# llm-d/llm-d-workload-variant-autoscaler

Measured on AMD Instinct MI355X. Metric: desired-replica accuracy + SLO-attainment %, Llama-3-8B synthetic QPS ramp, higher is better.
Workload: dtype bf16; 1 GPU; model=meta-llama/Llama-3.1-8B, global_batch=256, seq_len=150, parallelism=dp1, device=AMD Radeon Graphics

## Files before the change

### wva_amd/calibration/model.py

```python
from __future__ import annotations

import math
from dataclasses import dataclass
from typing import List, Optional

import torch

from .. import ops


@dataclass
class LlamaConfig:
    name: str = "llama"
    hidden_size: int = 4096
    intermediate_size: int = 14336
    num_layers: int = 32
    num_q_heads: int = 32
    num_kv_heads: int = 8
    head_dim: int = 128
    vocab_size: int = 128256
    rope_theta: float = 500000.0
    rms_eps: float = 1e-5

    @property
# ... 144 lines not shown
        self.context_lens[:batch] = context_len
        for layer in range(self.cfg.num_layers):
            if self.cache_dtype == torch.bfloat16:
                self.k_cache[layer][:batch, :, :context_len].normal_(0.0, 1.0)
                self.v_cache[layer][:batch, :, :context_len].normal_(0.0, 1.0)
            else:
                shape = self.k_cache[layer][:batch, :, :context_len].shape
                for cache in (self.k_cache, self.v_cache):
                    cache[layer][:batch, :, :context_len] = torch.randn(
                        shape, device=self.device, dtype=torch.bfloat16
                    ).to(self.cache_dtype)

    def _linear(self, x: torch.Tensor, layer, name: str) -> torch.Tensor:
        if self.weights_dtype == "bf16":
            w = getattr(layer, name) if layer is not None else self.lm_head
            return ops.linear(x, w)
        w8, w_scale = (
            getattr(layer, name + "_q") if layer is not None else self.lm_head_q
        )
        if not x.is_cuda:
            return (
                x.float() @ (w8.float() * w_scale[:, None]).t()
            ).to(x.dtype)
        if x.shape[0] <= 64 and x.shape[1] % 128 == 0:
            from .. import ops as _ops

            return _ops._require_ext().skinny_linear_fp8(x, w8, w_scale)
        return (x @ (w8.to(x.dtype) * w_scale[:, None].to(x.dtype)).t())

    @torch.no_grad()
    def decode_step(self, token_ids: torch.Tensor) -> torch.Tensor:
        cfg = self.cfg
        B = token_ids.shape[0]
        positions = self.context_lens[:B].clone()

        ctx = positions + 1
        x = self.embed.index_select(0, token_ids)
        residual: Optional[torch.Tensor] = None

        for li, layer in enumerate(self.layers):
            if residual is None:
                residual = x.clone()
                h = ops.rmsnorm(x, layer.input_norm, None, cfg.rms_eps)
            else:
                h = ops.rmsnorm(x, layer.input_norm, residual, cfg.rms_eps)

            qkv = self._linear(h, layer, "wqkv")
            q = ops.rope_append_kv(
                qkv, self.k_cache[li][:B], self.v_cache[li][:B],
                positions, cfg.num_q_heads, cfg.num_kv_heads, cfg.rope_theta,
            )

            attn = ops.gqa_decode_attn(
                q, self.k_cache[li][:B], self.v_cache[li][:B], ctx, self.scale
            )
            x = self._linear(attn.reshape(B, cfg.q_size), layer, "wo")

            h2 = ops.rmsnorm(x, layer.post_attn_norm, residual, cfg.rms_eps)
            gate_up = self._linear(h2, layer, "w_gate_up")
            act = ops.silu_mul_fused(gate_up)
            x = self._linear(act, layer, "w_down")

        final = ops.rmsnorm(x, self.final_norm, residual, cfg.rms_eps)
        logits = self._linear(final, None, "lm_head")
        self.context_lens[:B] += 1
        return logits

    @torch.no_grad()
    def prefill(self, token_ids: torch.Tensor) -> torch.Tensor:
        cfg = self.cfg
        if self.weights_dtype != "bf16":
            raise NotImplementedError(
                "prefill with fp8 weights is not implemented (the "
                "weight-only fp8 mode targets decode; prefill would "
                "dequantize every layer per pass)"
            )
        B, S = token_ids.shape
        T = B * S
        if S > self.max_seq:
            raise ValueError(f"S={S} exceeds max_seq={self.max_seq}")
        positions = (
            torch.arange(S, device=self.device, dtype=torch.int32)
            .repeat(B)
        )

        x = self.embed.index_select(0, token_ids.reshape(-1))
        residual: Optional[torch.Tensor] = None

# ... 73 lines not shown
```

### wva_amd/ops/__init__.py

```python
from __future__ import annotations

import glob
import importlib.util
import math
import os
from typing import Optional

import torch

_HERE = os.path.dirname(os.path.abspath(__file__))
_ext = None
_ext_error: Optional[str] = None


def _try_load_extension():
    global _ext, _ext_error
    if _ext is not None:
        return _ext
    candidates = sorted(glob.glob(os.path.join(_HERE, "_wva_ops*.so")))
    if not candidates:
        _ext_error = (
            f"HIP extension _wva_ops*.so not found in {_HERE}; build it with "
            "`python -m wva_amd.ops.build` (or __graft_entry__.build())"
        )
# ... 152 lines not shown
    idx = torch.arange(B)
    k_cache[idx, :, positions.long()] = k.to(k_cache.dtype)
    v_cache[idx, :, positions.long()] = v.to(v_cache.dtype)
    return q


def silu_mul_fused(gate_up: torch.Tensor) -> torch.Tensor:
    if gate_up.is_cuda:
        return _require_ext().silu_mul_fused(gate_up)
    inter = gate_up.shape[1] // 2
    return silu_mul_ref(gate_up[:, :inter], gate_up[:, inter:]).to(
        gate_up.dtype
    )


def gqa_decode_attn(
    q: torch.Tensor,
    k_cache: torch.Tensor,
    v_cache: torch.Tensor,
    context_lens: torch.Tensor,
    scale: Optional[float] = None,
) -> torch.Tensor:
    if scale is None:
        scale = 1.0 / math.sqrt(q.shape[-1])
    if q.is_cuda:
        return _require_ext().gqa_decode_attn(
            q, k_cache, v_cache, context_lens.to(torch.int32), scale
        )
    return gqa_decode_attn_ref(q, k_cache, v_cache, context_lens, scale).to(
        q.dtype
    )


def enable_tuned_gemms() -> bool:
    import os as _os

    import torch as _torch

    path = _os.path.join(_os.path.dirname(__file__), "tunableop_gfx950.csv")
    if not _torch.cuda.is_available() or not _os.path.exists(path):
        return False
    tun = _torch.cuda.tunable
    tun.enable(True)
    tun.tuning_enable(False)
    tun.read_file(path)
    return True


def linear(x: torch.Tensor, w: torch.Tensor) -> torch.Tensor:
    if (
        os.environ.get("WVA_FORCE_SKINNY")
        and x.is_cuda
        and x.shape[0] <= 16
        and x.shape[1] % 128 == 0
        and x.shape[1] <= 8192
        and w.shape[0] <= 8192
    ):
        return _require_ext().skinny_linear(x, w)
    return x @ w.t()


def prefill_attn(
    q: torch.Tensor,
    k_cache: torch.Tensor,
    v_cache: torch.Tensor,
    batch: int,
# ... 5 lines not shown
```

### wva_amd/ops/csrc/attention.hip

```cpp
#include "common.h"

#define HEAD_DIM 128
#define MAX_G 8
#define TILE 64
#define NUM_WAVES 4
#define ROW_DW 66

typedef __attribute__((ext_vector_type(4))) unsigned int uint4_t;

__global__ __launch_bounds__(256, 2) void gqa_decode_attn_kernel(
    bf16* __restrict__ out,
    float* __restrict__ workspace,
    const bf16* __restrict__ q,
    const bf16* __restrict__ k_cache,
    const bf16* __restrict__ v_cache,
    const int* __restrict__ context_lens,
    const int num_q_heads,
    const int num_kv_heads,
    const int max_seq,
    const float scale) {
  const int b = blockIdx.x;
  const int kvh = blockIdx.y;
  const int split = blockIdx.z;
  const int num_splits = gridDim.z;
// ... 126 lines not shown
        wsp[0] = m[j];
        wsp[1] = s[j];
      }
      wsp[2 + 2 * lane] = acc[j][0];
      wsp[2 + 2 * lane + 1] = acc[j][1];
    }
  }
}


typedef __attribute__((ext_vector_type(8))) short bf16x8_frag;
typedef __attribute__((ext_vector_type(4))) float f32x4_frag;

__device__ __forceinline__ short f2bf_bits(float v) {
  const bf16 b = f2bf(v);
  return *reinterpret_cast<const short*>(&b);
}

__device__ __forceinline__ long pack8_fp8(const float* v, float inv_scale) {
  unsigned int lo = 0, hi = 0;
  lo = __builtin_amdgcn_cvt_pk_fp8_f32(v[0] * inv_scale, v[1] * inv_scale,
                                       lo, false);
  lo = __builtin_amdgcn_cvt_pk_fp8_f32(v[2] * inv_scale, v[3] * inv_scale,
                                       lo, true);
  hi = __builtin_amdgcn_cvt_pk_fp8_f32(v[4] * inv_scale, v[5] * inv_scale,
                                       hi, false);
  hi = __builtin_amdgcn_cvt_pk_fp8_f32(v[6] * inv_scale, v[7] * inv_scale,
                                       hi, true);
  return (long)(((unsigned long)hi << 32) | lo);
}

#define S_ROW 65

template <bool KV_FP8>
__global__ __launch_bounds__(256, 2) void gqa_decode_attn_v4_kernel(
    bf16* __restrict__ out,
    float* __restrict__ workspace,
    const bf16* __restrict__ q,
    const void* __restrict__ k_cache,
    const void* __restrict__ v_cache,
    const int* __restrict__ context_lens,
    const int num_q_heads,
    const int num_kv_heads,
    const int max_seq,
    const float scale) {
  const int b = blockIdx.x;
  const int kvh = blockIdx.y;
  const int split = blockIdx.z;
  const int num_splits = gridDim.z;
  const int G = num_q_heads / num_kv_heads;
  const int ctx = context_lens[b];

  const int lane = threadIdx.x & (WAVE_SIZE - 1);
  const int wave = threadIdx.x / WAVE_SIZE;

  __shared__ float s_smem[MAX_G][S_ROW];
  __shared__ unsigned int v_smem[TILE * ROW_DW];
  __shared__ float p_smem[MAX_G][TILE];

  bf16x8_frag q_frag[4];
  long q8_frag[4] = {0, 0, 0, 0};
  float q_scale = 1.0f;
  {
    const int g = lane % 16;
    const int k0 = 8 * (lane / 16);
    float qv[4][8];
#pragma unroll
    for (int kk = 0; kk < 4; ++kk)
#pragma unroll
      for (int i = 0; i < 8; ++i) qv[kk][i] = 0.0f;
    if (g < G) {
      const bf16* qrow = q + ((long)b * num_q_heads + kvh * G + g) * HEAD_DIM;
#pragma unroll
      for (int kk = 0; kk < 4; ++kk) {
        const short* src = reinterpret_cast<const short*>(qrow + 32 * kk + k0);
#pragma unroll
        for (int i = 0; i < 8; ++i) {
          q_frag[kk][i] = src[i];
          const bf16 bv = *reinterpret_cast<const bf16*>(&src[i]);
          qv[kk][i] = bf2f(bv);
        }
      }
    } else {
#pragma unroll
      for (int kk = 0; kk < 4; ++kk)
#pragma unroll
        for (int i = 0; i < 8; ++i) q_frag[kk][i] = 0;
    }
    if constexpr (KV_FP8) {
      float amax = 0.0f;
#pragma unroll
      for (int kk = 0; kk < 4; ++kk)
#pragma unroll
        for (int i = 0; i < 8; ++i) amax = fmaxf(amax, fabsf(qv[kk][i]));
      amax = wave_reduce_max(amax);
      __shared__ float qmax_smem[NUM_WAVES];
      if (lane == 0) qmax_smem[wave] = amax;
      __syncthreads();
      float m0 = qmax_smem[0];
#pragma unroll
      for (int w2 = 1; w2 < NUM_WAVES; ++w2) m0 = fmaxf(m0, qmax_smem[w2]);
      q_scale = fmaxf(m0 / 448.0f, 1e-12f);
      const float inv = 1.0f / q_scale;
#pragma unroll
      for (int kk = 0; kk < 4; ++kk) q8_frag[kk] = pack8_fp8(qv[kk], inv);
      __syncthreads();
    }
  }

  const int heads_mine = (G > wave) ? (G - wave + NUM_WAVES - 1) / NUM_WAVES : 0;
  float m[2], s[2], acc[2][2];
#pragma unroll
  for (int j = 0; j < 2; ++j) {
    m[j] = -INFINITY;
    s[j] = 0.0f;
    acc[j][0] = acc[j][1] = 0.0f;
  }

  const long kv_row_dw = HEAD_DIM / 2;
  const long slab_off = ((long)b * num_kv_heads + kvh) * max_seq * HEAD_DIM;
  const bf16* k_slab = reinterpret_cast<const bf16*>(k_cache) + slab_off;
  const fp8_t* k_slab8 = reinterpret_cast<const fp8_t*>(k_cache) + slab_off;
  const unsigned int* v_base = reinterpret_cast<const unsigned int*>(
      reinterpret_cast<const bf16*>(v_cache) + slab_off);
  const fp8_t* v_base8 = reinterpret_cast<const fp8_t*>(v_cache) + slab_off;

  for (int t0 = split * TILE; t0 < ctx; t0 += num_splits * TILE) {
    const int tn = min(TILE, ctx - t0);

    if constexpr (KV_FP8) {
      const int tile_g8 = tn * (HEAD_DIM / 8);
      const fp8_t* v_src = v_base8 + (long)t0 * HEAD_DIM;
      for (int idx = wave * WAVE_SIZE + lane; idx < tile_g8;
           idx += NUM_WAVES * WAVE_SIZE) {
        const int row = idx >> 4;
        const int d8 = (idx & 15) * 8;
        const unsigned short* src =
            reinterpret_cast<const unsigned short*>(
                v_src + (long)row * HEAD_DIM + d8);
        unsigned int* dst = &v_smem[row * ROW_DW + d8 / 2];
#pragma unroll
        for (int j = 0; j < 4; ++j) {
          const float2_vt f = unpk2_fp8(src[j]);
          const bf16x2 packed{f2bf(f[0]), f2bf(f[1])};
          dst[j] = *reinterpret_cast<const unsigned int*>(&packed);
        }
      }
    } else {
      typedef __attribute__((ext_vector_type(2))) unsigned int uint2_t;
      const int tile_u2 = tn * (HEAD_DIM / 4);
      const unsigned int* v_src = &v_base[(long)t0 * kv_row_dw];
      for (int idx = wave * WAVE_SIZE + lane; idx < tile_u2;
           idx += NUM_WAVES * WAVE_SIZE) {
        const int row = idx >> 5;
        const int d2 = (idx & 31) * 2;
        const uint2_t val = *reinterpret_cast<const uint2_t*>(&v_src[idx * 2]);
        *reinterpret_cast<uint2_t*>(&v_smem[row * ROW_DW + d2]) = val;
      }
// ... 53 lines not shown
      acc[j][1] *= corr;
      m[j] = m_new;
      p_smem[g][lane] = p;
    }

    for (int j = 0; j < heads_mine; ++j) {
      const int g = wave + j * NUM_WAVES;
      const float* pg = p_smem[g];
      float a0 = acc[j][0], a1 = acc[j][1];
      for (int t = 0; t < tn; ++t) {
        const unsigned int vw = v_smem[t * ROW_DW + lane];
        const bf16x2 vv = *reinterpret_cast<const bf16x2*>(&vw);
        const float p = pg[t];
        a0 = fmaf(p, bf2f(vv.x), a0);
        a1 = fmaf(p, bf2f(vv.y), a1);
      }
      acc[j][0] = a0;
      acc[j][1] = a1;
    }
    __syncthreads();
  }

  if (num_splits == 1) {
    for (int j = 0; j < heads_mine; ++j) {
      const int g = wave + j * NUM_WAVES;
      const float inv = s[j] > 0.0f ? 1.0f / s[j] : 0.0f;
      bf16x2* orow = reinterpret_cast<bf16x2*>(
          out + ((long)b * num_q_heads + kvh * G + g) * HEAD_DIM);
      orow[lane] = bf16x2{f2bf(acc[j][0] * inv), f2bf(acc[j][1] * inv)};
    }
  } else {
    for (int j = 0; j < heads_mine; ++j) {
      const int g = wave + j * NUM_WAVES;
      float* wsp = workspace +
          ((((long)b * num_kv_heads + kvh) * G + g) * num_splits + split) *
              (2 + HEAD_DIM);
      if (lane == 0) {
        wsp[0] = m[j];
        wsp[1] = s[j];
      }
      wsp[2 + 2 * lane] = acc[j][0];
      wsp[2 + 2 * lane + 1] = acc[j][1];
    }
  }
}


template <bool KV_FP8>
__global__ __launch_bounds__(256, 2) void gqa_decode_attn_v5_kernel(
    bf16* __restrict__ out,
    float* __restrict__ workspace,
    const bf16* __restrict__ q,
    const void* __restrict__ k_cache,
    const void* __restrict__ v_cache,
    const int* __restrict__ context_lens,
    const int num_q_heads,
    const int num_kv_heads,
    const int max_seq,
    const float scale) {
  const int b = blockIdx.x;
  const int kvh = blockIdx.y;
  const int split = blockIdx.z;
  const int num_splits = gridDim.z;
  const int G = num_q_heads / num_kv_heads;
  const int ctx = context_lens[b];

  const int lane = threadIdx.x & (WAVE_SIZE - 1);
  const int wave = threadIdx.x / WAVE_SIZE;

  __shared__ float s_smem[MAX_G][S_ROW];
  __shared__ unsigned int v_smem[TILE * ROW_DW];
  __shared__ float p_smem[MAX_G][TILE];
  __shared__ float corr_smem[MAX_G];
  __shared__ float sum_smem[MAX_G];
  __shared__ float m_smem[MAX_G];

  bf16x8_frag q_frag[4];
  long q8_frag[4] = {0, 0, 0, 0};
  float q_scale = 1.0f;
  {
    const int g = lane % 16;
    const int k0 = 8 * (lane / 16);
    float qv[4][8];
#pragma unroll
    for (int kk = 0; kk < 4; ++kk)
#pragma unroll
      for (int i = 0; i < 8; ++i) qv[kk][i] = 0.0f;
    if (g < G) {
      const bf16* qrow = q + ((long)b * num_q_heads + kvh * G + g) * HEAD_DIM;
#pragma unroll
      for (int kk = 0; kk < 4; ++kk) {
        const short* src = reinterpret_cast<const short*>(qrow + 32 * kk + k0);
#pragma unroll
        for (int i = 0; i < 8; ++i) {
          q_frag[kk][i] = src[i];
          const bf16 bv = *reinterpret_cast<const bf16*>(&src[i]);
          qv[kk][i] = bf2f(bv);
        }
      }
    } else {
#pragma unroll
      for (int kk = 0; kk < 4; ++kk)
#pragma unroll
        for (int i = 0; i < 8; ++i) q_frag[kk][i] = 0;
    }
    if constexpr (KV_FP8) {
      float amax = 0.0f;
#pragma unroll
      for (int kk = 0; kk < 4; ++kk)
#pragma unroll
        for (int i = 0; i < 8; ++i) amax = fmaxf(amax, fabsf(qv[kk][i]));
      amax = wave_reduce_max(amax);
      __shared__ float qmax_smem5[NUM_WAVES];
      if (lane == 0) qmax_smem5[wave] = amax;
      __syncthreads();
      float m0 = qmax_smem5[0];
#pragma unroll
      for (int w2 = 1; w2 < NUM_WAVES; ++w2) m0 = fmaxf(m0, qmax_smem5[w2]);
      q_scale = fmaxf(m0 / 448.0f, 1e-12f);
      const float inv = 1.0f / q_scale;
#pragma unroll
      for (int kk = 0; kk < 4; ++kk) q8_frag[kk] = pack8_fp8(qv[kk], inv);
      __syncthreads();
    }
  }

  const int heads_mine = (G > wave) ? (G - wave + NUM_WAVES - 1) / NUM_WAVES : 0;
  float m[2], s[2];
#pragma unroll
  for (int j = 0; j < 2; ++j) {
    m[j] = -INFINITY;
    s[j] = 0.0f;
  }
  f32x4_frag acc_pv[2] = {f32x4_frag{0.f, 0.f, 0.f, 0.f},
                          f32x4_frag{0.f, 0.f, 0.f, 0.f}};

  const long kv_row_dw = HEAD_DIM / 2;
  const long slab_off = ((long)b * num_kv_heads + kvh) * max_seq * HEAD_DIM;
  const bf16* k_slab = reinterpret_cast<const bf16*>(k_cache) + slab_off;
  const fp8_t* k_slab8 = reinterpret_cast<const fp8_t*>(k_cache) + slab_off;
  const unsigned int* v_base = reinterpret_cast<const unsigned int*>(
      reinterpret_cast<const bf16*>(v_cache) + slab_off);
  const fp8_t* v_base8 = reinterpret_cast<const fp8_t*>(v_cache) + slab_off;

  for (int t0 = split * TILE; t0 < ctx; t0 += num_splits * TILE) {
    const int tn = min(TILE, ctx - t0);

    if constexpr (KV_FP8) {
      const int tile_g8 = tn * (HEAD_DIM / 8);
      const fp8_t* v_src = v_base8 + (long)t0 * HEAD_DIM;
      for (int idx = wave * WAVE_SIZE + lane; idx < tile_g8;
           idx += NUM_WAVES * WAVE_SIZE) {
        const int row = idx >> 4;
        const int d8 = (idx & 15) * 8;
        const unsigned short* src =
            reinterpret_cast<const unsigned short*>(
                v_src + (long)row * HEAD_DIM + d8);
        unsigned int* dst = &v_smem[row * ROW_DW + d8 / 2];
#pragma unroll
        for (int j = 0; j < 4; ++j) {
          const float2_vt f = unpk2_fp8(src[j]);
          const bf16x2 packed{f2bf(f[0]), f2bf(f[1])};
          dst[j] = *reinterpret_cast<const unsigned int*>(&packed);
        }
      }
    } else {
      typedef __attribute__((ext_vector_type(2))) unsigned int uint2_t;
      const int tile_u2 = tn * (HEAD_DIM / 4);
      const unsigned int* v_src = &v_base[(long)t0 * kv_row_dw];
      for (int idx = wave * WAVE_SIZE + lane; idx < tile_u2;
           idx += NUM_WAVES * WAVE_SIZE) {
        const int row = idx >> 5;
        const int d2 = (idx & 31) * 2;
        const uint2_t val = *reinterpret_cast<const uint2_t*>(&v_src[idx * 2]);
        *reinterpret_cast<uint2_t*>(&v_smem[row * ROW_DW + d2]) = val;
      }
// ... 102 lines not shown
  }

  for (int j = 0; j < heads_mine; ++j) {
    const int g = wave + j * NUM_WAVES;
    if (lane == 0) {
      sum_smem[g] = s[j];
      m_smem[g] = m[j];
    }
  }
  __syncthreads();

  if (num_splits == 1) {
#pragma unroll
    for (int nsub = 0; nsub < 2; ++nsub) {
      const int dim = 16 * (wave + 4 * nsub) + (lane & 15);
#pragma unroll
      for (int i = 0; i < 4; ++i) {
        const int h = (lane >> 4) * 4 + i;
        if (h >= G) continue;
        const float sv = sum_smem[h];
        const float inv = sv > 0.0f ? 1.0f / sv : 0.0f;
        out[((long)b * num_q_heads + kvh * G + h) * HEAD_DIM + dim] =
            f2bf(acc_pv[nsub][i] * inv);
      }
    }
  } else {
#pragma unroll
    for (int nsub = 0; nsub < 2; ++nsub) {
      const int dim = 16 * (wave + 4 * nsub) + (lane & 15);
#pragma unroll
      for (int i = 0; i < 4; ++i) {
        const int h = (lane >> 4) * 4 + i;
        if (h >= G) continue;
        float* wsp = workspace +
            ((((long)b * num_kv_heads + kvh) * G + h) * num_splits + split) *
                (2 + HEAD_DIM);
        if (wave == 0 && nsub == 0 && (lane & 15) == 0) {
          wsp[0] = m_smem[h];
          wsp[1] = sum_smem[h];
        }
        wsp[2 + dim] = acc_pv[nsub][i];
      }
    }
  }
}

#define MERGE_WAVES 8
__global__ __launch_bounds__(64 * MERGE_WAVES) void gqa_decode_attn_merge_kernel(
    bf16* __restrict__ out,
    const float* __restrict__ workspace,
    const int num_q_heads,
    const int num_kv_heads,
    const int num_splits) {
  const int b = blockIdx.x;
  const int h = blockIdx.y;
  const int G = num_q_heads / num_kv_heads;
  const int kvh = h / G;
  const int g = h % G;
  const int lane = threadIdx.x & 63;
  const int wave = threadIdx.x >> 6;

  __shared__ float sm_m[MERGE_WAVES];
  __shared__ float sm_s[MERGE_WAVES];
  __shared__ float sm_o[MERGE_WAVES][HEAD_DIM];

  const float* base = workspace +
      ((((long)b * num_kv_heads + kvh) * G + g) * (long)num_splits) *
          (2 + HEAD_DIM);
  float M = -INFINITY;
  for (int sp = wave; sp < num_splits; sp += MERGE_WAVES) {
    M = fmaxf(M, base[sp * (2 + HEAD_DIM)]);
  }
  float S = 0.0f, o0 = 0.0f, o1 = 0.0f;
  for (int sp = wave; sp < num_splits; sp += MERGE_WAVES) {
    const float* wsp = base + sp * (2 + HEAD_DIM);
// ... 72 lines not shown
  hipLaunchKernelGGL(gqa_decode_attn_kernel, grid, block, 0, stream,
                     (bf16*)out, (float*)workspace, (const bf16*)q,
                     (const bf16*)k_cache, (const bf16*)v_cache, context_lens,
                     num_q_heads, num_kv_heads, max_seq, scale);
  if (num_splits > 1) {
    dim3 mgrid(batch, num_q_heads);
    hipLaunchKernelGGL(gqa_decode_attn_merge_kernel, mgrid, dim3(64 * MERGE_WAVES), 0,
                       stream, (bf16*)out, (const float*)workspace,
                       num_q_heads, num_kv_heads, num_splits);
  }
}

extern "C" void launch_gqa_decode_attn_v5(
    void* out, void* workspace, const void* q, const void* k_cache,
    const void* v_cache, const int* context_lens, int batch, int num_q_heads,
    int num_kv_heads, int max_seq, int num_splits, float scale,
    hipStream_t stream) {
  launch_gqa_decode_attn_v5_ex(out, workspace, q, k_cache, v_cache,
                               context_lens, batch, num_q_heads, num_kv_heads,
                               max_seq, num_splits, scale, 0, stream);
}

extern "C" void launch_gqa_decode_attn_v5_ex(
    void* out, void* workspace, const void* q, const void* k_cache,
    const void* v_cache, const int* context_lens, int batch, int num_q_heads,
    int num_kv_heads, int max_seq, int num_splits, float scale, int kv_fp8,
    hipStream_t stream) {
  dim3 grid(batch, num_kv_heads, num_splits);
  dim3 block(256);
  if (kv_fp8) {
    hipLaunchKernelGGL(gqa_decode_attn_v5_kernel<true>, grid, block, 0,
                       stream, (bf16*)out, (float*)workspace, (const bf16*)q,
                       k_cache, v_cache, context_lens, num_q_heads,
                       num_kv_heads, max_seq, scale);
  } else {
    hipLaunchKernelGGL(gqa_decode_attn_v5_kernel<false>, grid, block, 0,
                       stream, (bf16*)out, (float*)workspace, (const bf16*)q,
                       k_cache, v_cache, context_lens, num_q_heads,
                       num_kv_heads, max_seq, scale);
  }
  if (num_splits > 1) {
    dim3 mgrid(batch, num_q_heads);
    hipLaunchKernelGGL(gqa_decode_attn_merge_kernel, mgrid, dim3(64 * MERGE_WAVES), 0,
                       stream, (bf16*)out, (const float*)workspace,
                       num_q_heads, num_kv_heads, num_splits);
  }
}

extern "C" void launch_gqa_decode_attn_v4(
    void* out, void* workspace, const void* q, const void* k_cache,
    const void* v_cache, const int* context_lens, int batch, int num_q_heads,
    int num_kv_heads, int max_seq, int num_splits, float scale,
    hipStream_t stream) {
  launch_gqa_decode_attn_v4_ex(out, workspace, q, k_cache, v_cache,
                               context_lens, batch, num_q_heads, num_kv_heads,
                               max_seq, num_splits, scale, 0, stream);
}

extern "C" void launch_gqa_decode_attn_v4_ex(
    void* out, void* workspace, const void* q, const void* k_cache,
    const void* v_cache, const int* context_lens, int batch, int num_q_heads,
    int num_kv_heads, int max_seq, int num_splits, float scale, int kv_fp8,
    hipStream_t stream) {
  dim3 grid(batch, num_kv_heads, num_splits);
  dim3 block(256);
  if (kv_fp8) {
    hipLaunchKernelGGL(gqa_decode_attn_v4_kernel<true>, grid, block, 0,
                       stream, (bf16*)out, (float*)workspace, (const bf16*)q,
                       k_cache, v_cache, context_lens, num_q_heads,
                       num_kv_heads, max_seq, scale);
  } else {
    hipLaunchKernelGGL(gqa_decode_attn_v4_kernel<false>, grid, block, 0,
                       stream, (bf16*)out, (float*)workspace, (const bf16*)q,
                       k_cache, v_cache, context_lens, num_q_heads,
                       num_kv_heads, max_seq, scale);
  }
  if (num_splits > 1) {
    dim3 mgrid(batch, num_q_heads);
    hipLaunchKernelGGL(gqa_decode_attn_merge_kernel, mgrid, dim3(64 * MERGE_WAVES), 0,
                       stream, (bf16*)out, (const float*)workspace,
                       num_q_heads, num_kv_heads, num_splits);
  }
}
```

### wva_amd/ops/csrc/ops.cpp

```cpp

#include <torch/extension.h>
#include <hip/hip_runtime.h>
#include <c10/hip/HIPStream.h>

extern "C" void launch_rmsnorm(void* out, void* residual_out,
                               const void* input, const void* residual,
                               const void* weight, float eps, int rows,
                               int hidden, hipStream_t stream);
extern "C" void launch_rope(void* q, void* k, const int* positions, int tokens,
                            int num_q_heads, int num_k_heads, int head_dim,
                            float theta, hipStream_t stream);
extern "C" void launch_silu_mul(void* out, const void* gate, const void* up,
                                long n, hipStream_t stream);
extern "C" void launch_silu_mul_fused(void* out, const void* gate_up,
                                      long rows, long inter,
                                      hipStream_t stream);
extern "C" void launch_rope_append_kv_fp8(const void* qkv, void* q_out,
                                          void* k_cache, void* v_cache,
                                          const int* positions, int batch,
                                          int num_q_heads, int num_kv_heads,
                                          int head_dim, int max_seq,
                                          float theta, hipStream_t stream);
extern "C" void launch_gqa_decode_attn_v4_ex(void* out, void* workspace,
                                             const void* q,
                                             const void* k_cache,
                                             const void* v_cache,
                                             const int* context_lens,
                                             int batch, int num_q_heads,
                                             int num_kv_heads, int max_seq,
                                             int num_splits, float scale,
                                             int kv_fp8, hipStream_t stream);
extern "C" void launch_gqa_decode_attn_v5_ex(void* out, void* workspace,
                                             const void* q,
                                             const void* k_cache,
                                             const void* v_cache,
                                             const int* context_lens,
                                             int batch, int num_q_heads,
                                             int num_kv_heads, int max_seq,
                                             int num_splits, float scale,
                                             int kv_fp8, hipStream_t stream);
extern "C" void launch_rope_append_kv(const void* qkv, void* q_out,
                                      void* k_cache, void* v_cache,
                                      const int* positions, int batch,
                                      int num_q_heads, int num_kv_heads,
                                      int head_dim, int max_seq, float theta,
                                      hipStream_t stream);
extern "C" int gqa_decode_attn_num_splits(int batch, int num_kv_heads,
                                          int max_ctx_hint);
extern "C" int skinny_gemm_num_splits(int N, int K, int nt);
extern "C" void launch_prefill_attn_ex(void* out, const void* q,
                                       const void* k_cache,
                                       const void* v_cache, int batch,
                                       int seq, int num_q_heads,
                                       int num_kv_heads, int max_seq,
                                       float scale, int kv_fp8,
                                       hipStream_t stream);
extern "C" int skinny_gemm_tile_n(int M);
extern "C" void launch_skinny_gemm(void* c, void* ws, const void* a,
                                   const void* w, int M, int N, int K,
                                   int num_splits, hipStream_t stream);
extern "C" void launch_skinny_gemm_ex(void* c, void* ws, const void* a,
                                      const void* w, const float* w_scale,
                                      int M, int N, int K, int num_splits,
                                      int w_fp8, hipStream_t stream);
extern "C" void launch_gqa_decode_attn(void* out, void* workspace,
                                       const void* q, const void* k_cache,
                                       const void* v_cache,
                                       const int* context_lens, int batch,
                                       int num_q_heads, int num_kv_heads,
                                       int max_seq, int num_splits,
                                       float scale, hipStream_t stream);
extern "C" void launch_gqa_decode_attn_v5(void* out, void* workspace,
                                          const void* q, const void* k_cache,
                                          const void* v_cache,
                                          const int* context_lens, int batch,
                                          int num_q_heads, int num_kv_heads,
                                          int max_seq, int num_splits,
                                          float scale, hipStream_t stream);
extern "C" void launch_gqa_decode_attn_v4(void* out, void* workspace,
// ... 166 lines not shown
           k_cache.data_ptr(), v_cache.data_ptr(),
           context_lens.data_ptr<int>(), batch, num_q_heads,
           num_kv_heads, max_seq, num_splits, (float)scale,
           kv_fp8 ? 1 : 0, current_stream());
  }
  return out;
}

torch::Tensor gqa_decode_attn(torch::Tensor q, torch::Tensor k_cache,
                              torch::Tensor v_cache,
                              torch::Tensor context_lens, double scale) {
  const int G = (int)(q.size(1) / k_cache.size(1));
  const int splits = gqa_decode_attn_num_splits(
      (int)q.size(0), (int)k_cache.size(1), (int)k_cache.size(2));
  const int variant = (G >= 8 || splits == 1) ? 2 : 1;
  return gqa_decode_attn_impl(q, k_cache, v_cache, context_lens, scale,
                              variant);
}

torch::Tensor gqa_decode_attn_v5(torch::Tensor q, torch::Tensor k_cache,
                                 torch::Tensor v_cache,
                                 torch::Tensor context_lens, double scale) {
  return gqa_decode_attn_impl(q, k_cache, v_cache, context_lens, scale,
                              2);
}

torch::Tensor gqa_decode_attn_v3(torch::Tensor q, torch::Tensor k_cache,
                                 torch::Tensor v_cache,
                                 torch::Tensor context_lens, double scale) {
  return gqa_decode_attn_impl(q, k_cache, v_cache, context_lens, scale,
                              0);
}

torch::Tensor skinny_linear(torch::Tensor x, torch::Tensor w) {
  check_bf16_contig(x, "x");
  check_bf16_contig(w, "w");
  TORCH_CHECK(x.dim() == 2 && w.dim() == 2, "x [M,K], w [N,K]");
  const int M = x.size(0);
  const int K = x.size(1);
  const int N = w.size(0);
  TORCH_CHECK(w.size(1) == K, "K mismatch");
  TORCH_CHECK(M <= 64, "skinny_linear requires M <= 64");
  TORCH_CHECK(K % 128 == 0, "K must be a multiple of 128");
  auto y = torch::empty({M, N}, x.options());
  const int nt = skinny_gemm_tile_n(M);
  const int sk = skinny_gemm_num_splits(N, K, nt);
  torch::Tensor ws;
  void* ws_ptr = nullptr;
  if (sk > 1) {
    ws = torch::empty({(long)sk * M * N},
                      x.options().dtype(torch::kFloat32));
    ws_ptr = ws.data_ptr();
  }
  launch_skinny_gemm(y.data_ptr(), ws_ptr, x.data_ptr(), w.data_ptr(), M, N,
                     K, sk, current_stream());
  return y;
}

torch::Tensor skinny_linear_fp8(torch::Tensor x, torch::Tensor w,
                                torch::Tensor w_scale) {
  check_bf16_contig(x, "x");
  TORCH_CHECK(w.is_cuda() && w.is_contiguous() &&
                  w.scalar_type() == at::kFloat8_e4m3fn,
              "w must be contiguous float8_e4m3fn");
  TORCH_CHECK(w_scale.is_cuda() && w_scale.scalar_type() == torch::kFloat &&
                  w_scale.numel() == w.size(0),
// ... 56 lines not shown
        py::arg("theta") = 500000.0);
  m.def("silu_mul", &silu_mul, "Fused SwiGLU silu(gate)*up",
        py::arg("gate"), py::arg("up"));
  m.def("silu_mul_fused", &silu_mul_fused,
        "SwiGLU on the fused [rows, 2*inter] gate_up buffer",
        py::arg("gate_up"));
  m.def("rope_append_kv", &rope_append_kv,
        "RoPE on strided qkv row + KV-cache append; returns contiguous q",
        py::arg("qkv"), py::arg("k_cache"), py::arg("v_cache"),
        py::arg("positions"), py::arg("num_q_heads"), py::arg("num_kv_heads"),
        py::arg("theta") = 500000.0);
  m.def("gqa_decode_attn", &gqa_decode_attn,
        "GQA decode attention over contiguous KV cache",
        py::arg("q"), py::arg("k_cache"), py::arg("v_cache"),
        py::arg("context_lens"), py::arg("scale"));
  m.def("gqa_decode_attn_v4", &gqa_decode_attn,
        "GQA decode attention, MFMA-scores variant (= default)",
        py::arg("q"), py::arg("k_cache"), py::arg("v_cache"),
        py::arg("context_lens"), py::arg("scale"));
  m.def("prefill_attn", &prefill_attn,
        "Causal flash-attention prefill over head-major KV caches",
        py::arg("q"), py::arg("k_cache"), py::arg("v_cache"),
        py::arg("batch"), py::arg("seq"), py::arg("scale"));
  m.def("skinny_linear_fp8", &skinny_linear_fp8,
        "Weight-only fp8 decode GEMM: x[M,K]bf16 @ w[N,K]e4m3^T, M <= 64",
        py::arg("x"), py::arg("w"), py::arg("w_scale"));
  m.def("skinny_linear", &skinny_linear,
        "Weight-streaming decode GEMM: x[M,K] @ w[N,K]^T, M <= 64",
        py::arg("x"), py::arg("w"));
  m.def("gqa_decode_attn_v5", &gqa_decode_attn_v5,
        "GQA decode attention, MFMA scores + MFMA PV variant",
        py::arg("q"), py::arg("k_cache"), py::arg("v_cache"),
        py::arg("context_lens"), py::arg("scale"));
  m.def("gqa_decode_attn_v3", &gqa_decode_attn_v3,
        "GQA decode attention, pre-MFMA shared-tile variant",
        py::arg("q"), py::arg("k_cache"), py::arg("v_cache"),
        py::arg("context_lens"), py::arg("scale"));
}
```

Measured before the change: 91.98 %.

## Fuse RoPE and KV-cache append into the GQA decode attention kernel

Adds a fused decode path in which the attention kernel applies RoPE to Q in its prologue, and the split owning the new position writes the rotated K and the V row into the cache. This removes the separate rope_append_kv launch and the positions clone and add per layer. An optional level 2 also merges the splits inside the same launch through an atomic ticket counter, at the cost of a persistent counter buffer and relaxed-atomic workspace stores. Level 1 is the default for bf16 KV caches. The main risks are ordering and visibility between the split that writes the cache and the splits that read that row.

```diff
diff --git a/wva_amd/calibration/model.py b/wva_amd/calibration/model.py
--- a/wva_amd/calibration/model.py
+++ b/wva_amd/calibration/model.py
@@ -200,9 +200,13 @@
     def decode_step(self, token_ids: torch.Tensor) -> torch.Tensor:
         cfg = self.cfg
         B = token_ids.shape[0]
-        positions = self.context_lens[:B].clone()
-
-        ctx = positions + 1
+        fused_level = (
+            ops.fused_attn_level() if self.kv_dtype == "bf16" else 0
+        )
+        positions = self.context_lens[:B]
+        if fused_level == 0:
+            positions = positions.clone()
+            ctx = positions + 1
         x = self.embed.index_select(0, token_ids)
         residual: Optional[torch.Tensor] = None
 
@@ -214,14 +218,22 @@
                 h = ops.rmsnorm(x, layer.input_norm, residual, cfg.rms_eps)
 
             qkv = self._linear(h, layer, "wqkv")
-            q = ops.rope_append_kv(
-                qkv, self.k_cache[li][:B], self.v_cache[li][:B],
-                positions, cfg.num_q_heads, cfg.num_kv_heads, cfg.rope_theta,
-            )
-
-            attn = ops.gqa_decode_attn(
-                q, self.k_cache[li][:B], self.v_cache[li][:B], ctx, self.scale
-            )
+            if fused_level != 0:
+                attn = ops.fused_rope_attn(
+                    qkv, self.k_cache[li][:B], self.v_cache[li][:B],
+                    positions, cfg.num_q_heads, cfg.num_kv_heads,
+                    cfg.rope_theta, self.scale, fused_level,
+                )
+            else:
+                q = ops.rope_append_kv(
+                    qkv, self.k_cache[li][:B], self.v_cache[li][:B],
+                    positions, cfg.num_q_heads, cfg.num_kv_heads,
+                    cfg.rope_theta,
+                )
+                attn = ops.gqa_decode_attn(
+                    q, self.k_cache[li][:B], self.v_cache[li][:B], ctx,
+                    self.scale,
+                )
             x = self._linear(attn.reshape(B, cfg.q_size), layer, "wo")
 
             h2 = ops.rmsnorm(x, layer.post_attn_norm, residual, cfg.rms_eps)
diff --git a/wva_amd/ops/__init__.py b/wva_amd/ops/__init__.py
--- a/wva_amd/ops/__init__.py
+++ b/wva_amd/ops/__init__.py
@@ -208,6 +208,54 @@
     )
 
 
+FUSED_ATTN_DEFAULT = 1
+_fused_attn_level: Optional[int] = None
+
+
+def fused_attn_level() -> int:
+    global _fused_attn_level
+    if _fused_attn_level is None:
+        raw = os.environ.get("WVA_FUSED_ATTN")
+        level = FUSED_ATTN_DEFAULT if raw in (None, "") else int(raw)
+        if level not in (0, 1, 2):
+            raise ValueError(f"WVA_FUSED_ATTN must be 0, 1 or 2, got {raw!r}")
+        _fused_attn_level = level
+    return _fused_attn_level
+
+
+def set_fused_attn_level(level: Optional[int]) -> None:
+    global _fused_attn_level
+    if level is not None and level not in (0, 1, 2):
+        raise ValueError(f"level must be 0, 1, 2 or None, got {level!r}")
+    _fused_attn_level = level
+
+
+def fused_rope_attn(
+    qkv: torch.Tensor,
+    k_cache: torch.Tensor,
+    v_cache: torch.Tensor,
+    positions: torch.Tensor,
+    num_q_heads: int,
+    num_kv_heads: int,
+    theta: float = 500000.0,
+    scale: Optional[float] = None,
+    level: Optional[int] = None,
+) -> torch.Tensor:
+    if scale is None:
+        scale = 1.0 / math.sqrt(k_cache.shape[-1])
+    if level is None:
+        level = fused_attn_level()
+    if qkv.is_cuda and level != 0:
+        return _require_ext().fused_rope_attn(
+            qkv, k_cache, v_cache, positions.to(torch.int32),
+            num_q_heads, num_kv_heads, theta, scale, level,
+        )
+    q = rope_append_kv(
+        qkv, k_cache, v_cache, positions, num_q_heads, num_kv_heads, theta
+    )
+    return gqa_decode_attn(q, k_cache, v_cache, positions + 1, scale)
+
+
 def enable_tuned_gemms() -> bool:
     import os as _os
 
diff --git a/wva_amd/ops/csrc/attention.hip b/wva_amd/ops/csrc/attention.hip
--- a/wva_amd/ops/csrc/attention.hip
+++ b/wva_amd/ops/csrc/attention.hip
@@ -182,7 +182,143 @@
 
 #define S_ROW 65
 
-template <bool KV_FP8>
+struct FusedArgs {
+  const bf16* qkv;
+  bf16* k_cache;
+  bf16* v_cache;
+  float* workspace;
+  int* counters;
+  float theta;
+};
+
+__device__ __forceinline__ void fused_rope_prologue(
+    bf16x8_frag (&q_frag)[4], const FusedArgs& fa, float* cs, const int b,
+    const int kvh, const int G, const int num_q_heads, const int num_kv_heads,
+    const int max_seq, const int pos_i, const bool owner, const int lane,
+    const int wave) {
+  const float pos = (float)pos_i;
+  const long qkv_row =
+      (long)b * (num_q_heads + 2 * num_kv_heads) * HEAD_DIM;
+  float c = 0.0f, s = 0.0f;
+  if (wave == 0) {
+    const int d = lane;
+    const float inv_freq =
+        __powf(fa.theta, -2.0f * (float)d / (float)HEAD_DIM);
+    const float angle = pos * inv_freq;
+    __sincosf(angle, &s, &c);
+    cs[d] = c;
+    cs[64 + d] = s;
+  }
+  __syncthreads();
+  {
+    const int g = lane % 16;
+    const int k0 = 8 * (lane / 16);
+    if (g < G) {
+      const bf16* qrow = fa.qkv + qkv_row + (long)(kvh * G + g) * HEAD_DIM;
+#pragma unroll
+      for (int kk = 0; kk < 2; ++kk) {
+        const int d0 = 32 * kk + k0;
+        const bf16* lo = qrow + d0;
+        const bf16* hi = qrow + d0 + HEAD_DIM / 2;
+#pragma unroll
+        for (int i = 0; i < 8; ++i) {
+          const float cd = cs[d0 + i];
+          const float sd = cs[64 + d0 + i];
+          const float x1 = bf2f(lo[i]);
+          const float x2 = bf2f(hi[i]);
+          q_frag[kk][i] = f2bf_bits(x1 * cd - x2 * sd);
+          q_frag[kk + 2][i] = f2bf_bits(x2 * cd + x1 * sd);
+        }
+      }
+    } else {
+#pragma unroll
+      for (int kk = 0; kk < 4; ++kk)
+#pragma unroll
+        for (int i = 0; i < 8; ++i) q_frag[kk][i] = 0;
+    }
+  }
+  if (owner) {
+    const long dst_off =
+        (((long)b * num_kv_heads + kvh) * max_seq + pos_i) * HEAD_DIM;
+    if (wave == 0) {
+      const int d = lane;
+      const bf16* src =
+          fa.qkv + qkv_row + (long)(num_q_heads + kvh) * HEAD_DIM;
+      bf16* dst = fa.k_cache + dst_off;
+      const float x1 = bf2f(src[d]);
+      const float x2 = bf2f(src[d + HEAD_DIM / 2]);
+      dst[d] = f2bf(x1 * c - x2 * s);
+      dst[d + HEAD_DIM / 2] = f2bf(x2 * c + x1 * s);
+    } else if (wave == 1) {
+      const bf16x2* vsrc = reinterpret_cast<const bf16x2*>(
+          fa.qkv + qkv_row +
+          (long)(num_q_heads + num_kv_heads + kvh) * HEAD_DIM);
+      reinterpret_cast<bf16x2*>(fa.v_cache + dst_off)[lane] = vsrc[lane];
+    }
+    asm volatile("s_waitcnt vmcnt(0)" ::: "memory");
+    __syncthreads();
+  }
+}
+
+template <int FUSED>
+__device__ __forceinline__ void ws_store(float* p, const float v) {
+  if constexpr (FUSED == 2) {
+    __hip_atomic_store(p, v, __ATOMIC_RELAXED, __HIP_MEMORY_SCOPE_AGENT);
+  } else {
+    *p = v;
+  }
+}
+
+__device__ __forceinline__ void fused_merge_tail(
+    bf16* __restrict__ out, const FusedArgs& fa, int* flag, const int b,
+    const int kvh, const int G, const int num_q_heads, const int num_kv_heads,
+    const int num_splits, const int lane, const int wave) {
+  asm volatile("s_waitcnt vmcnt(0)" ::: "memory");
+  __syncthreads();
+  if (threadIdx.x == 0) {
+    int* cnt = fa.counters + b * num_kv_heads + kvh;
+    const int ticket = __hip_atomic_fetch_add(cnt, 1, __ATOMIC_RELAXED,
+                                              __HIP_MEMORY_SCOPE_AGENT);
+    const int last = ticket == num_splits - 1;
+    if (last) {
+      __hip_atomic_store(cnt, 0, __ATOMIC_RELAXED, __HIP_MEMORY_SCOPE_AGENT);
+      __builtin_amdgcn_fence(__ATOMIC_ACQUIRE, "agent");
+      asm volatile("s_waitcnt vmcnt(0)" ::: "memory");
+    }
+    *flag = last;
+  }
+  __syncthreads();
+  if (*flag == 0) return;
+
+  typedef __attribute__((ext_vector_type(2))) float float2_t;
+  for (int g = wave; g < G; g += NUM_WAVES) {
+    const float* base = fa.workspace +
+        ((((long)b * num_kv_heads + kvh) * G + g) * (long)num_splits) *
+            (2 + HEAD_DIM);
+    float M = -INFINITY;
+    for (int sp = 0; sp < num_splits; ++sp)
+      M = fmaxf(M, base[sp * (2 + HEAD_DIM)]);
+    float S = 0.0f, o0 = 0.0f, o1 = 0.0f;
+#pragma unroll 4
+    for (int sp = 0; sp < num_splits; ++sp) {
+      const float* wsp = base + sp * (2 + HEAD_DIM);
+      const float mw = wsp[0];
+      if (mw == -INFINITY) continue;
+      const float f = __expf(mw - M);
+      const float2_t a =
+          *reinterpret_cast<const float2_t*>(&wsp[2 + 2 * lane]);
+      S += wsp[1] * f;
+      o0 = fmaf(a[0], f, o0);
+      o1 = fmaf(a[1], f, o1);
+    }
+    const float inv = S > 0.0f ? 1.0f / S : 0.0f;
+    bf16x2* orow = reinterpret_cast<bf16x2*>(
+        out + ((long)b * num_q_heads + kvh * G + g) * HEAD_DIM);
+    orow[lane] = bf16x2{f2bf(o0 * inv), f2bf(o1 * inv)};
+  }
+}
+
+template <bool KV_FP8, int FUSED = 0>
 __global__ __launch_bounds__(256, 2) void gqa_decode_attn_v4_kernel(
     bf16* __restrict__ out,
     float* __restrict__ workspace,
@@ -193,13 +329,15 @@
     const int num_q_heads,
     const int num_kv_heads,
     const int max_seq,
-    const float scale) {
+    const float scale,
+    const FusedArgs fa) {
+  static_assert(!(KV_FP8 && FUSED), "fused entry is bf16-cache only");
   const int b = blockIdx.x;
   const int kvh = blockIdx.y;
   const int split = blockIdx.z;
   const int num_splits = gridDim.z;
   const int G = num_q_heads / num_kv_heads;
-  const int ctx = context_lens[b];
+  const int ctx = FUSED ? context_lens[b] + 1 : context_lens[b];
 
   const int lane = threadIdx.x & (WAVE_SIZE - 1);
   const int wave = threadIdx.x / WAVE_SIZE;
@@ -211,7 +349,12 @@
   bf16x8_frag q_frag[4];
   long q8_frag[4] = {0, 0, 0, 0};
   float q_scale = 1.0f;
-  {
+  if constexpr (FUSED != 0) {
+    const int pos_i = ctx - 1;
+    fused_rope_prologue(q_frag, fa, &p_smem[0][0], b, kvh, G, num_q_heads,
+                        num_kv_heads, max_seq, pos_i,
+                        split == (pos_i / TILE) % num_splits, lane, wave);
+  } else {
     const int g = lane % 16;
     const int k0 = 8 * (lane / 16);
     float qv[4][8];
@@ -269,11 +412,14 @@
 
   const long kv_row_dw = HEAD_DIM / 2;
   const long slab_off = ((long)b * num_kv_heads + kvh) * max_seq * HEAD_DIM;
-  const bf16* k_slab = reinterpret_cast<const bf16*>(k_cache) + slab_off;
+  const bf16* k_slab =
+      (FUSED ? fa.k_cache : reinterpret_cast<const bf16*>(k_cache)) + slab_off;
   const fp8_t* k_slab8 = reinterpret_cast<const fp8_t*>(k_cache) + slab_off;
   const unsigned int* v_base = reinterpret_cast<const unsigned int*>(
-      reinterpret_cast<const bf16*>(v_cache) + slab_off);
+      (FUSED ? fa.v_cache : reinterpret_cast<const bf16*>(v_cache)) +
+      slab_off);
   const fp8_t* v_base8 = reinterpret_cast<const fp8_t*>(v_cache) + slab_off;
+  float* const ws = FUSED ? fa.workspace : workspace;
 
   for (int t0 = split * TILE; t0 < ctx; t0 += num_splits * TILE) {
     const int tn = min(TILE, ctx - t0);
@@ -393,21 +539,26 @@
   } else {
     for (int j = 0; j < heads_mine; ++j) {
       const int g = wave + j * NUM_WAVES;
-      float* wsp = workspace +
+      float* wsp = ws +
           ((((long)b * num_kv_heads + kvh) * G + g) * num_splits + split) *
               (2 + HEAD_DIM);
       if (lane == 0) {
-        wsp[0] = m[j];
-        wsp[1] = s[j];
-      }
-      wsp[2 + 2 * lane] = acc[j][0];
-      wsp[2 + 2 * lane + 1] = acc[j][1];
-    }
-  }
-}
-
-
-template <bool KV_FP8>
+        ws_store<FUSED>(&wsp[0], m[j]);
+        ws_store<FUSED>(&wsp[1], s[j]);
+      }
+      ws_store<FUSED>(&wsp[2 + 2 * lane], acc[j][0]);
+      ws_store<FUSED>(&wsp[2 + 2 * lane + 1], acc[j][1]);
+    }
+    if constexpr (FUSED == 2) {
+      fused_merge_tail(out, fa, reinterpret_cast<int*>(&p_smem[0][0]), b,
+                       kvh, G, num_q_heads, num_kv_heads, num_splits, lane,
+                       wave);
+    }
+  }
+}
+
+
+template <bool KV_FP8, int FUSED = 0>
 __global__ __launch_bounds__(256, 2) void gqa_decode_attn_v5_kernel(
     bf16* __restrict__ out,
     float* __restrict__ workspace,
@@ -418,13 +569,15 @@
     const int num_q_heads,
     const int num_kv_heads,
     const int max_seq,
-    const float scale) {
+    const float scale,
+    const FusedArgs fa) {
+  static_assert(!(KV_FP8 && FUSED), "fused entry is bf16-cache only");
   const int b = blockIdx.x;
   const int kvh = blockIdx.y;
   const int split = blockIdx.z;
   const int num_splits = gridDim.z;
   const int G = num_q_heads / num_kv_heads;
-  const int ctx = context_lens[b];
+  const int ctx = FUSED ? context_lens[b] + 1 : context_lens[b];
 
   const int lane = threadIdx.x & (WAVE_SIZE - 1);
   const int wave = threadIdx.x / WAVE_SIZE;
@@ -439,7 +592,12 @@
   bf16x8_frag q_frag[4];
   long q8_frag[4] = {0, 0, 0, 0};
   float q_scale = 1.0f;
-  {
+  if constexpr (FUSED != 0) {
+    const int pos_i = ctx - 1;
+    fused_rope_prologue(q_frag, fa, &p_smem[0][0], b, kvh, G, num_q_heads,
+                        num_kv_heads, max_seq, pos_i,
+                        split == (pos_i / TILE) % num_splits, lane, wave);
+  } else {
     const int g = lane % 16;
     const int k0 = 8 * (lane / 16);
     float qv[4][8];
@@ -498,11 +656,14 @@
 
   const long kv_row_dw = HEAD_DIM / 2;
   const long slab_off = ((long)b * num_kv_heads + kvh) * max_seq * HEAD_DIM;
-  const bf16* k_slab = reinterpret_cast<const bf16*>(k_cache) + slab_off;
+  const bf16* k_slab =
+      (FUSED ? fa.k_cache : reinterpret_cast<const bf16*>(k_cache)) + slab_off;
   const fp8_t* k_slab8 = reinterpret_cast<const fp8_t*>(k_cache) + slab_off;
   const unsigned int* v_base = reinterpret_cast<const unsigned int*>(
-      reinterpret_cast<const bf16*>(v_cache) + slab_off);
+      (FUSED ? fa.v_cache : reinterpret_cast<const bf16*>(v_cache)) +
+      slab_off);
   const fp8_t* v_base8 = reinterpret_cast<const fp8_t*>(v_cache) + slab_off;
+  float* const ws = FUSED ? fa.workspace : workspace;
 
   for (int t0 = split * TILE; t0 < ctx; t0 += num_splits * TILE) {
     const int tn = min(TILE, ctx - t0);
@@ -671,15 +832,20 @@
       for (int i = 0; i < 4; ++i) {
         const int h = (lane >> 4) * 4 + i;
         if (h >= G) continue;
-        float* wsp = workspace +
+        float* wsp = ws +
             ((((long)b * num_kv_heads + kvh) * G + h) * num_splits + split) *
                 (2 + HEAD_DIM);
         if (wave == 0 && nsub == 0 && (lane & 15) == 0) {
-          wsp[0] = m_smem[h];
-          wsp[1] = sum_smem[h];
-        }
-        wsp[2 + dim] = acc_pv[nsub][i];
-      }
+          ws_store<FUSED>(&wsp[0], m_smem[h]);
+          ws_store<FUSED>(&wsp[1], sum_smem[h]);
+        }
+        ws_store<FUSED>(&wsp[2 + dim], acc_pv[nsub][i]);
+      }
+    }
+    if constexpr (FUSED == 2) {
+      fused_merge_tail(out, fa, reinterpret_cast<int*>(&p_smem[0][0]), b,
+                       kvh, G, num_q_heads, num_kv_heads, num_splits, lane,
+                       wave);
     }
   }
 }
@@ -818,12 +984,12 @@
     hipLaunchKernelGGL(gqa_decode_attn_v5_kernel<true>, grid, block, 0,
                        stream, (bf16*)out, (float*)workspace, (const bf16*)q,
                        k_cache, v_cache, context_lens, num_q_heads,
-                       num_kv_heads, max_seq, scale);
+                       num_kv_heads, max_seq, scale, FusedArgs{});
   } else {
     hipLaunchKernelGGL(gqa_decode_attn_v5_kernel<false>, grid, block, 0,
                        stream, (bf16*)out, (float*)workspace, (const bf16*)q,
                        k_cache, v_cache, context_lens, num_q_heads,
-                       num_kv_heads, max_seq, scale);
+                       num_kv_heads, max_seq, scale, FusedArgs{});
   }
   if (num_splits > 1) {
     dim3 mgrid(batch, num_q_heads);
@@ -854,12 +1020,12 @@
     hipLaunchKernelGGL(gqa_decode_attn_v4_kernel<true>, grid, block, 0,
                        stream, (bf16*)out, (float*)workspace, (const bf16*)q,
                        k_cache, v_cache, context_lens, num_q_heads,
-                       num_kv_heads, max_seq, scale);
+                       num_kv_heads, max_seq, scale, FusedArgs{});
   } else {
     hipLaunchKernelGGL(gqa_decode_attn_v4_kernel<false>, grid, block, 0,
                        stream, (bf16*)out, (float*)workspace, (const bf16*)q,
                        k_cache, v_cache, context_lens, num_q_heads,
-                       num_kv_heads, max_seq, scale);
+                       num_kv_heads, max_seq, scale, FusedArgs{});
   }
   if (num_splits > 1) {
     dim3 mgrid(batch, num_q_heads);
@@ -868,3 +1034,43 @@
                        num_q_heads, num_kv_heads, num_splits);
   }
 }
+
+extern "C" void launch_fused_rope_attn(
+    void* out, void* workspace, int* counters, const void* qkv, void* k_cache,
+    void* v_cache, const int* positions, int batch, int num_q_heads,
+    int num_kv_heads, int max_seq, int num_splits, float theta, float scale,
+    int variant, int level, hipStream_t stream) {
+  dim3 grid(batch, num_kv_heads, num_splits);
+  dim3 block(256);
+  const FusedArgs fa{(const bf16*)qkv, (bf16*)k_cache, (bf16*)v_cache,
+                     (float*)workspace, counters, theta};
+  const bool in_launch_merge = level == 2 && num_splits > 1;
+  bf16* o = (bf16*)out;
+  if (variant == 2) {
+    if (in_launch_merge) {
+      gqa_decode_attn_v5_kernel<false, 2><<<grid, block, 0, stream>>>(
+          o, nullptr, nullptr, nullptr, nullptr, positions, num_q_heads,
+          num_kv_heads, max_seq, scale, fa);
+    } else {
+      gqa_decode_attn_v5_kernel<false, 1><<<grid, block, 0, stream>>>(
+          o, nullptr, nullptr, nullptr, nullptr, positions, num_q_heads,
+          num_kv_heads, max_seq, scale, fa);
+    }
+  } else {
+    if (in_launch_merge) {
+      gqa_decode_attn_v4_kernel<false, 2><<<grid, block, 0, stream>>>(
+          o, nullptr, nullptr, nullptr, nullptr, positions, num_q_heads,
+          num_kv_heads, max_seq, scale, fa);
+    } else {
+      gqa_decode_attn_v4_kernel<false, 1><<<grid, block, 0, stream>>>(
+          o, nullptr, nullptr, nullptr, nullptr, positions, num_q_heads,
+          num_kv_heads, max_seq, scale, fa);
+    }
+  }
+  if (num_splits > 1 && !in_launch_merge) {
+    dim3 mgrid(batch, num_q_heads);
+    hipLaunchKernelGGL(gqa_decode_attn_merge_kernel, mgrid, dim3(64 * MERGE_WAVES), 0,
+                       stream, (bf16*)out, (const float*)workspace,
+                       num_q_heads, num_kv_heads, num_splits);
+  }
+}
diff --git a/wva_amd/ops/csrc/ops.cpp b/wva_amd/ops/csrc/ops.cpp
--- a/wva_amd/ops/csrc/ops.cpp
+++ b/wva_amd/ops/csrc/ops.cpp
@@ -2,6 +2,11 @@
 #include <torch/extension.h>
 #include <hip/hip_runtime.h>
 #include <c10/hip/HIPStream.h>
+
+#include <algorithm>
+#include <mutex>
+#include <unordered_map>
+#include <vector>
 
 extern "C" void launch_rmsnorm(void* out, void* residual_out,
                                const void* input, const void* residual,
@@ -45,6 +50,14 @@
                                       int num_q_heads, int num_kv_heads,
                                       int head_dim, int max_seq, float theta,
                                       hipStream_t stream);
+extern "C" void launch_fused_rope_attn(void* out, void* workspace,
+                                       int* counters, const void* qkv,
+                                       void* k_cache, void* v_cache,
+                                       const int* positions, int batch,
+                                       int num_q_heads, int num_kv_heads,
+                                       int max_seq, int num_splits,
+                                       float theta, float scale, int variant,
+                                       int level, hipStream_t stream);
 extern "C" int gqa_decode_attn_num_splits(int batch, int num_kv_heads,
                                           int max_ctx_hint);
 extern "C" int skinny_gemm_num_splits(int N, int K, int nt);
@@ -277,6 +290,91 @@
                               0);
 }
 
+int* fused_attn_counters(const torch::Tensor& like, long needed) {
+  static std::mutex mu;
+  static std::unordered_map<int, std::vector<torch::Tensor>> bufs;
+  std::lock_guard<std::mutex> lock(mu);
+  auto& v = bufs[like.get_device()];
+  if (v.empty() || v.back().numel() < needed) {
+    hipStreamCaptureStatus st = hipStreamCaptureStatusNone;
+    TORCH_CHECK(hipStreamIsCapturing(current_stream(), &st) == hipSuccess &&
+                    st == hipStreamCaptureStatusNone,
+                "fused_rope_attn: the split-merge counter buffer must be "
+                "created by an eager call before graph capture");
+    const long n = std::max<long>(needed, 16384);
+    v.push_back(torch::zeros({n}, like.options().dtype(torch::kInt32)));
+  }
+  return v.back().data_ptr<int>();
+}
+
+torch::Tensor fused_rope_attn_impl(torch::Tensor qkv, torch::Tensor k_cache,
+                                   torch::Tensor v_cache,
+                                   torch::Tensor positions,
+                                   int64_t num_q_heads, int64_t num_kv_heads,
+                                   double theta, double scale, int64_t level,
+                                   int64_t variant, int64_t force_splits) {
+  check_bf16_contig(qkv, "qkv");
+  TORCH_CHECK(!check_cache_contig(k_cache, "k_cache") &&
+                  !check_cache_contig(v_cache, "v_cache"),
+              "fused_rope_attn supports bf16 KV caches only; use "
+              "rope_append_kv + gqa_decode_attn for fp8 caches");
+  TORCH_CHECK(positions.is_cuda() && positions.is_contiguous() &&
+                  positions.scalar_type() == torch::kInt32,
+              "positions must be contiguous int32 on GPU");
+  TORCH_CHECK(qkv.dim() == 2, "qkv must be [B, (Hq+2Hk)*D]");
+  TORCH_CHECK(k_cache.dim() == 4,
+              "k_cache must be [B, Hk, S, D] (head-major)");
+  TORCH_CHECK(v_cache.sizes() == k_cache.sizes(), "k/v cache mismatch");
+  const int batch = qkv.size(0);
+  const int head_dim = k_cache.size(3);
+  const int max_seq = k_cache.size(2);
+  TORCH_CHECK(head_dim == 128, "head_dim must be 128 (Llama-3 family)");
+  TORCH_CHECK(k_cache.size(0) >= batch && positions.numel() >= batch,
+              "batch mismatch");
+  TORCH_CHECK(k_cache.size(1) == num_kv_heads, "Hk mismatch");
+  TORCH_CHECK(qkv.size(1) == (num_q_heads + 2 * num_kv_heads) * head_dim,
+              "qkv width mismatch");
+  TORCH_CHECK(num_q_heads % num_kv_heads == 0, "Hq must divide by Hk");
+  const int G = num_q_heads / num_kv_heads;
+  TORCH_CHECK(G <= 8, "GQA group size must be <= 8");
+  TORCH_CHECK(level == 1 || level == 2, "level must be 1 or 2");
+  TORCH_CHECK(variant >= 0 && variant <= 2, "variant must be 0, 1 or 2");
+  TORCH_CHECK(force_splits >= 0 && force_splits <= 65535,
+              "force_splits out of range");
+  const int num_splits =
+      force_splits > 0
+          ? (int)force_splits
+          : gqa_decode_attn_num_splits(batch, (int)num_kv_heads, max_seq);
+  if (variant == 0) variant = (G >= 8 || num_splits == 1) ? 2 : 1;
+  auto out = torch::empty({batch, num_q_heads, head_dim}, qkv.options());
+  torch::Tensor workspace;
+  void* ws_ptr = nullptr;
+  int* counters = nullptr;
+  if (num_splits > 1) {
+    workspace = torch::empty(
+        {(long)batch * num_kv_heads * G * num_splits * (2 + head_dim)},
+        qkv.options().dtype(torch::kFloat32));
+    ws_ptr = workspace.data_ptr();
+    if (level == 2)
+      counters = fused_attn_counters(qkv, (long)batch * num_kv_heads);
+  }
+  launch_fused_rope_attn(out.data_ptr(), ws_ptr, counters, qkv.data_ptr(),
+                         k_cache.data_ptr(), v_cache.data_ptr(),
+                         positions.data_ptr<int>(), batch, (int)num_q_heads,
+                         (int)num_kv_heads, max_seq, num_splits, (float)theta,
+                         (float)scale, (int)variant, (int)level,
+                         current_stream());
+  return out;
+}
+
+torch::Tensor fused_rope_attn(torch::Tensor qkv, torch::Tensor k_cache,
+                              torch::Tensor v_cache, torch::Tensor positions,
+                              int64_t num_q_heads, int64_t num_kv_heads,
+                              double theta, double scale, int64_t level) {
+  return fused_rope_attn_impl(qkv, k_cache, v_cache, positions, num_q_heads,
+                              num_kv_heads, theta, scale, level, 0, 0);
+}
+
 torch::Tensor skinny_linear(torch::Tensor x, torch::Tensor w) {
   check_bf16_contig(x, "x");
   check_bf16_contig(w, "w");
@@ -399,6 +497,17 @@
         "GQA decode attention, MFMA scores + MFMA PV variant",
         py::arg("q"), py::arg("k_cache"), py::arg("v_cache"),
         py::arg("context_lens"), py::arg("scale"));
+  m.def("fused_rope_attn", &fused_rope_attn,
+        "RoPE + KV append + GQA decode attention (+ split merge), bf16 KV",
+        py::arg("qkv"), py::arg("k_cache"), py::arg("v_cache"),
+        py::arg("positions"), py::arg("num_q_heads"), py::arg("num_kv_heads"),
+        py::arg("theta"), py::arg("scale"), py::arg("level") = 1);
+  m.def("fused_rope_attn_ex", &fused_rope_attn_impl,
+        "fused_rope_attn with forced kernel variant / split count (tests)",
+        py::arg("qkv"), py::arg("k_cache"), py::arg("v_cache"),
+        py::arg("positions"), py::arg("num_q_heads"), py::arg("num_kv_heads"),
+        py::arg("theta"), py::arg("scale"), py::arg("level"),
+        py::arg("variant"), py::arg("force_splits"));
   m.def("gqa_decode_attn_v3", &gqa_decode_attn_v3,
         "GQA decode attention, pre-MFMA shared-tile variant",
         py::arg("q"), py::arg("k_cache"), py::arg("v_cache"),
```

Result: no change. 91.98 % (+0.0%).
